# maturk/dn-splatter

Measured on NVIDIA H100. Metric: rendered Mpix/s (fwd+bwd, RGB+depth+normal), higher is better.
Workload: dtype f32

## Files before the change

### dn_splatter_b200/_lib.py

```python
from __future__ import annotations

import ctypes as C
import os
from typing import Optional

HERE = os.path.dirname(os.path.abspath(__file__))
LIB_PATH = os.path.join(HERE, "libdnr_b200.so")

FLAG_ACTIVATED, FLAG_ANTIALIASED, FLAG_NORMALS, FLAG_ACCUMULATE, FLAG_EXACT_LISTS = 1, 2, 4, 8, 16
FLAG_HOST_CAMERA = 32
FLAG_PERSISTENT_WS = 256
LOSS_FUSED_BWD, LOSS_IMG_U8, LOSS_NORMAL_U8, LOSS_EDGE_FROM_IMAGE = 1, 2, 4, 8
REC_FLOATS, REC_FLOATS_N, GRAD_FLOATS = 12, 16, 16
DEPTH_LOSS_TYPES = {None: 0, "EdgeAwareLogL1": 1, "LogL1": 2, "L1": 3, "MSE": 4}

_f, _i, _p = C.c_float, C.c_int32, C.c_void_p


class DnrArgs(C.Structure):

    _fields_ = [
        ("n_gauss", _i), ("width", _i), ("height", _i), ("tile_size", _i), ("sh_degree", _i), ("sh_bases", _i),
        ("flags", C.c_uint32), ("list_shift", _i),
        ("near_plane", _f), ("far_plane", _f), ("eps2d", _f), ("radius_clip", _f),
        ("background", _f * 3), ("reserved1", _f),
        ("n_isects", C.c_int64),
        ("viewmat", _p), ("K", _p), ("c2w", _p),
        ("means", _p), ("quats", _p), ("scales", _p), ("opacities", _p), ("sh_dc", _p), ("sh_rest", _p),
        ("radii", _p), ("means2d", _p), ("depths", _p), ("conics", _p), ("opac_act", _p), ("compensations", _p),
        ("colors", _p), ("normals_world", _p), ("tiles_per_gauss", _p), ("depth_keys", _p), ("records", _p), ("cull_lim", _p),
        ("ws_scan", _p), ("ws_sort", _p), ("flatten_ids", _p), ("tile_offsets", _p), ("n_isects_dev", _p),
        ("out_rgb", _p), ("out_depth", _p), ("out_alpha", _p), ("out_normal", _p), ("out_surface_normal", _p),
        ("last_ids", _p), ("normal_norm", _p), ("clamp_mask", _p), ("depth_max", _p),
        ("v_rgb", _p), ("v_depth", _p), ("v_normal", _p), ("v_alpha", _p), ("grad_records", _p),
        ("v_means", _p), ("v_quats", _p), ("v_scales", _p), ("v_opacities", _p), ("v_sh_dc", _p), ("v_sh_rest", _p),
        ("v_means2d", _p), ("v_means2d_abs", _p),
        ("gt_depth", _p), ("gt_normal", _p), ("gt_rgb", _p), ("loss_partials", _p), ("v_loss", _p),
        ("depth_lambda", _f), ("depth_tolerance", _f), ("depth_loss_type", _i), ("use_normal_loss", _i),
        ("host_cam", _f * 32),
        ("reserved2", _p),
        ("loss_flags", C.c_uint32), ("reserved3", _i), ("gt_image", _p), ("v_l1", _p), ("touched", _p), ("stats", _p),
        ("v_viewmat", _p),
    ]


class DnrAdamSeg(C.Structure):

    _fields_ = [("p", _p), ("g", _p), ("m", _p), ("v", _p), ("n", C.c_int64), ("lr", C.c_double), ("eps", C.c_double),
                ("bc1", C.c_double), ("bc2_sqrt", C.c_double), ("dense", C.c_int64)]


class DnrGradSeg(C.Structure):

    _fields_ = [("g", _p), ("width", _i), ("dense", _i)]


PEER_MAX = 8


class DnrPeerReduce(C.Structure):

    _fields_ = [("world", _i), ("rank", _i), ("n_gauss", _i), ("reserved", _i), ("peer_flat", _p * PEER_MAX),
                ("peer_touched", _p * PEER_MAX), ("mask", _p)]


class DnrKnnGrid(C.Structure):

    _fields_ = [("lo", _f * 3), ("cell", _f), ("inv_cell", _f), ("dims", C.c_int32 * 3)]


class DnrTsdfGrid(C.Structure):

    _fields_ = [("origin", _f * 3), ("voxel", _f), ("sdf_trunc", _f), ("dims", C.c_int32 * 3), ("voxels", _p)]


class DnrMcField(C.Structure):

    _fields_ = [("values", _p), ("valid", _p), ("tsdf", _p), ("dims", C.c_int32 * 3), ("iso", _f), ("origin", _f * 3),
                ("spacing", _f)]


class DnrPoissonGrid(C.Structure):

    _fields_ = [("origin", _f * 3), ("cell", _f), ("depth", _i), ("reserved", _i)]


class DnrGridDesc(C.Structure):

    _fields_ = [("origin", _f * 3), ("cell", _f), ("dims", C.c_int32 * 3), ("channels", _i)]


POISSON_MIN_DEPTH, POISSON_MAX_DEPTH, POISSON_MAX_CYCLES = 4, 10, 100


POINTER_FIELDS = {n for n, t in DnrArgs._fields_ if t is _p}

_lib: Optional[C.CDLL] = None

KERNELS_PER_CALL = {
    "dnr_project_fwd": (1, 0), "dnr_bin_scan": (2, 8), "dnr_bin_sort": (3, 4), "dnr_raster_fwd": (1, 0),
    "dnr_finalize_fwd": (1, 0), "dnr_normal_from_depth": (1, 0), "dnr_raster_bwd": (1, 0), "dnr_project_bwd": (1, 0),
    "dnr_loss_fwd": (2, 0), "dnr_loss_bwd": (1, 0), "dnr_scale_loss_fwd": (1, 0), "dnr_scale_loss_bwd": (1, 0),
    "dnr_l1_fwd": (1, 0), "dnr_l1_bwd": (1, 0), "dnr_u8_to_f32": (1, 0),
    "dnr_ssim_fwd": (1, 0), "dnr_ssim_bwd": (1, 0), "dnr_ssim_fwd_ex": (1, 0), "dnr_ssim_bwd_ex": (1, 0), "dnr_photometric_fwd": (2, 0), "dnr_photometric_bwd": (1, 0), "dnr_adam_step": (1, 0), "dnr_adam_step_reduce": (2, 0),
    "dnr_grad_zero": (1, 0),
    "dnr_knn_build": (2, 1), "dnr_knn_query": (1, 0), "dnr_density": (1, 0), "dnr_ray_densities": (1, 0),
    "dnr_tsdf_integrate": (1, 0), "dnr_mc_count": (1, 6), "dnr_mc_emit": (2, 0),
    "dnr_grid_sample": (1, 0), "dnr_mesh_visibility": (1, 0),
}
LAUNCHES = {"handwritten": 0, "cub": 0}
DEBUG_CAPTURE = os.environ.get("DNR_DEBUG_CAPTURE") == "1"


def capture_ok(where: str) -> None:
    if not DEBUG_CAPTURE:
        return
    import torch

    try:
        torch.cuda.is_current_stream_capturing()
    except Exception as exc:
        raise DnrError(f"stream capture invalidated by {where}: {exc}") from exc


class _Counting:

    def __init__(self, lib):
        self._lib = lib

    def __getattr__(self, name):
        fn = getattr(self._lib, name)
        k = KERNELS_PER_CALL.get(name)
        if k is None:
            return fn

        def call(*args):
            LAUNCHES["handwritten"] += k[0]
            LAUNCHES["cub"] += k[1]
            rc = fn(*args)
            if DEBUG_CAPTURE:
                capture_ok(f"{name} (rc {rc})")
            return rc

        self.__dict__[name] = call
        return call


class DnrError(RuntimeError):
    pass


def load():
    global _lib
    if _lib is not None:
        return _lib
    if not os.path.exists(LIB_PATH):
        raise DnrError(
            f"{LIB_PATH} is missing: build it with `python -m dn_splatter_b200.build` "
            "(nvcc, sm_90a). dn_splatter_b200 has no CPU or PyTorch fallback."
        )
    lib = C.CDLL(LIB_PATH)
    A = C.POINTER(DnrArgs)
    lib.dnr_version.restype = C.c_int
    lib.dnr_error_string.restype = C.c_char_p
    lib.dnr_error_string.argtypes = [C.c_int]
    for name in ("dnr_project_fwd", "dnr_bin_sort", "dnr_raster_fwd", "dnr_finalize_fwd", "dnr_normal_from_depth",
                 "dnr_raster_bwd", "dnr_project_bwd", "dnr_loss_fwd"):
        fn = getattr(lib, name)
        fn.restype = C.c_int
        fn.argtypes = [A, C.c_void_p]
    lib.dnr_bin_scan.restype = C.c_int
    lib.dnr_bin_scan.argtypes = [A, C.c_void_p, C.POINTER(C.c_int64)]
    lib.dnr_loss_bwd.restype = C.c_int
    lib.dnr_loss_bwd.argtypes = [A, C.c_void_p, C.c_void_p, C.c_void_p]
    lib.dnr_scale_loss_fwd.restype = C.c_int
    lib.dnr_scale_loss_fwd.argtypes = [C.c_void_p, C.c_int32, C.c_void_p, C.c_void_p]
    lib.dnr_scale_loss_bwd.restype = C.c_int
    lib.dnr_scale_loss_bwd.argtypes = [C.c_void_p, C.c_int32, C.c_void_p, C.c_void_p, C.c_void_p]
    lib.dnr_l1_fwd.restype = C.c_int
    lib.dnr_l1_fwd.argtypes = [C.c_void_p, C.c_void_p, C.c_int64, C.c_int32, C.c_void_p, C.c_void_p]
    lib.dnr_l1_bwd.restype = C.c_int
    lib.dnr_l1_bwd.argtypes = [C.c_void_p, C.c_void_p, C.c_int64, C.c_int32, C.c_void_p, C.c_void_p, C.c_void_p]
    lib.dnr_u8_to_f32.restype = C.c_int
    lib.dnr_u8_to_f32.argtypes = [C.c_void_p, C.c_int64, C.c_float, C.c_float, C.c_void_p, C.c_void_p]
    lib.dnr_ssim_fwd.restype = C.c_int
    lib.dnr_ssim_fwd.argtypes = [C.c_void_p, C.c_void_p, C.c_int32, C.c_int32, C.c_int32, C.c_void_p, C.c_void_p, C.c_void_p]
    lib.dnr_ssim_fwd_ex.restype = C.c_int
    lib.dnr_ssim_fwd_ex.argtypes = [C.c_void_p, C.c_void_p, C.c_int32, C.c_int32, C.c_int32, C.c_int32, C.c_void_p, C.c_void_p,
                                    C.c_void_p]
    lib.dnr_ssim_bwd_ex.restype = C.c_int
    lib.dnr_ssim_bwd_ex.argtypes = [C.c_void_p, C.c_void_p, C.c_int32, C.c_int32, C.c_int32, C.c_int32, C.c_void_p, C.c_void_p,
                                    C.c_void_p, C.c_void_p]
    lib.dnr_photometric_fwd.restype = C.c_int
    lib.dnr_photometric_fwd.argtypes = [C.c_void_p, C.c_void_p, C.c_int32, C.c_int32, C.c_int32, C.c_int32, C.c_float, C.c_void_p,
                                        C.c_void_p, C.c_void_p]
    lib.dnr_photometric_bwd.restype = C.c_int
    lib.dnr_photometric_bwd.argtypes = [C.c_void_p, C.c_void_p, C.c_int32, C.c_int32, C.c_int32, C.c_int32, C.c_float, C.c_void_p,
                                        C.c_void_p, C.c_void_p, C.c_void_p]
    lib.dnr_adam_step.restype = C.c_int
    lib.dnr_adam_step.argtypes = [C.c_void_p, C.c_int32, C.c_double, C.c_double, C.c_void_p]
    lib.dnr_adam_step_reduce.restype = C.c_int
    lib.dnr_adam_step_reduce.argtypes = [C.c_void_p, C.c_void_p, C.c_int32, C.c_double, C.c_double, C.c_void_p, C.c_void_p]
    lib.dnr_grad_zero.restype = C.c_int
    lib.dnr_grad_zero.argtypes = [C.c_void_p, C.c_int32, C.c_void_p, C.c_int32, C.c_void_p]
    lib.dnr_knn_workspace_bytes.restype = C.c_int64
    lib.dnr_knn_workspace_bytes.argtypes = [C.c_int32, C.c_void_p]
    lib.dnr_knn_build.restype = C.c_int
    lib.dnr_knn_build.argtypes = [C.c_void_p, C.c_int32, C.c_void_p, C.c_void_p, C.c_int64, C.c_void_p]
    lib.dnr_knn_query.restype = C.c_int
    lib.dnr_knn_query.argtypes = [C.c_int32, C.c_void_p, C.c_void_p, C.c_void_p, C.c_int32, C.c_int32, C.c_int32, C.c_void_p,
                                  C.c_void_p, C.c_void_p]
    lib.dnr_density.restype = C.c_int
    lib.dnr_density.argtypes = [C.c_void_p, C.c_int64, C.c_void_p, C.c_int32, C.c_int32, C.c_void_p, C.c_void_p, C.c_void_p,
                                C.c_void_p, C.c_int32, C.c_float, C.c_void_p, C.c_void_p]
    lib.dnr_ray_densities.restype = C.c_int
    lib.dnr_ray_densities.argtypes = [C.c_void_p, C.c_int64, C.c_void_p, C.c_int32, C.c_void_p, C.c_void_p, C.c_void_p, C.c_void_p,
                                      C.c_void_p, C.c_int32, C.c_int32, C.c_float, C.c_void_p, C.c_void_p, C.c_void_p, C.c_void_p]
    lib.dnr_tsdf_integrate.restype = C.c_int
    lib.dnr_tsdf_integrate.argtypes = [C.c_void_p, C.c_void_p, C.c_void_p, C.c_void_p, C.c_int32, C.c_int32, C.c_void_p,
                                       C.c_float, C.c_void_p]
    lib.dnr_mc_count_workspace_bytes.restype = C.c_int64
    lib.dnr_mc_count_workspace_bytes.argtypes = [C.c_void_p]
    lib.dnr_mc_count.restype = C.c_int
    lib.dnr_mc_count.argtypes = [C.c_void_p, C.c_void_p, C.c_int64, C.c_void_p, C.c_void_p]
    lib.dnr_mc_emit_workspace_bytes.restype = C.c_int64
    lib.dnr_mc_emit_workspace_bytes.argtypes = [C.c_void_p]
    lib.dnr_mc_emit.restype = C.c_int
    lib.dnr_mc_emit.argtypes = [C.c_void_p, C.c_void_p, C.c_void_p, C.c_void_p, C.c_int64, C.c_void_p, C.c_void_p, C.c_void_p,
                                C.c_void_p]
    lib.dnr_poisson_splat_workspace_bytes.restype = C.c_int64
    lib.dnr_poisson_splat_workspace_bytes.argtypes = [C.c_void_p, C.c_int64]
    lib.dnr_poisson_splat.restype = C.c_int
    lib.dnr_poisson_splat.argtypes = [C.c_void_p, C.c_void_p, C.c_void_p, C.c_void_p, C.c_int64, C.c_void_p, C.c_int64,
                                      C.c_void_p, C.c_void_p, C.c_void_p, C.c_void_p, C.c_void_p, C.c_void_p, C.c_void_p]
    lib.dnr_poisson_solve_workspace_bytes.restype = C.c_int64
    lib.dnr_poisson_solve_workspace_bytes.argtypes = [C.c_void_p, C.c_int32]
    lib.dnr_poisson_solve.restype = C.c_int
    lib.dnr_poisson_solve.argtypes = [C.c_void_p, C.c_void_p, C.c_void_p, C.c_float, C.c_float, C.c_int32, C.c_void_p, C.c_int64,
                                      C.c_void_p, C.c_void_p, C.c_void_p, C.c_void_p]
    lib.dnr_grid_sample.restype = C.c_int
    lib.dnr_grid_sample.argtypes = [C.c_void_p, C.c_void_p, C.c_void_p, C.c_int64, C.c_void_p, C.c_void_p]
    lib.dnr_mesh_depth_workspace_bytes.restype = C.c_int64
    lib.dnr_mesh_depth_workspace_bytes.argtypes = [C.c_int64]
    lib.dnr_mesh_depth.restype = C.c_int
    lib.dnr_mesh_depth.argtypes = [C.c_void_p, C.c_int32, C.c_void_p, C.c_int64, C.c_void_p, C.c_int32, C.c_int32, C.c_int32,
                                   C.c_float, C.c_float, C.c_void_p, C.c_int64, C.c_void_p, C.c_void_p]
    lib.dnr_mesh_visibility.restype = C.c_int
    lib.dnr_mesh_visibility.argtypes = [C.c_void_p, C.c_int64, C.c_void_p, C.c_void_p, C.c_void_p, C.c_int32, C.c_int32, C.c_int32,
                                        C.c_float, C.c_void_p, C.c_void_p, C.c_void_p]
    lib.dnr_ssim_bwd.restype = C.c_int
    lib.dnr_ssim_bwd.argtypes = [C.c_void_p, C.c_void_p, C.c_int32, C.c_int32, C.c_int32, C.c_void_p, C.c_void_p, C.c_void_p,
                                 C.c_void_p]
    lib.dnr_bin_scan_workspace_bytes.restype = C.c_size_t
    lib.dnr_bin_scan_workspace_bytes.argtypes = [C.c_int32]
    lib.dnr_bin_sort_workspace_bytes.restype = C.c_size_t
    lib.dnr_bin_sort_workspace_bytes.argtypes = [C.c_int32, C.c_int64, C.c_int32]
    _lib = _Counting(lib)
    return _lib


EXPORTS = (
    "dnr_version", "dnr_error_string", "dnr_project_fwd", "dnr_bin_scan_workspace_bytes", "dnr_bin_scan",
    "dnr_bin_sort_workspace_bytes", "dnr_bin_sort", "dnr_raster_fwd", "dnr_finalize_fwd", "dnr_normal_from_depth",
    "dnr_raster_bwd", "dnr_project_bwd", "dnr_loss_fwd", "dnr_loss_bwd", "dnr_scale_loss_fwd", "dnr_scale_loss_bwd",
    "dnr_l1_fwd", "dnr_l1_bwd", "dnr_u8_to_f32", "dnr_ssim_fwd", "dnr_ssim_bwd", "dnr_ssim_fwd_ex", "dnr_ssim_bwd_ex", "dnr_photometric_fwd", "dnr_photometric_bwd", "dnr_adam_step", "dnr_adam_step_reduce", "dnr_grad_zero", "dnr_knn_workspace_bytes", "dnr_knn_build", "dnr_knn_query",
    "dnr_density", "dnr_ray_densities", "dnr_tsdf_integrate", "dnr_mc_count_workspace_bytes", "dnr_mc_count",
    "dnr_mc_emit_workspace_bytes", "dnr_mc_emit", "dnr_poisson_splat_workspace_bytes", "dnr_poisson_splat",
    "dnr_poisson_solve_workspace_bytes", "dnr_poisson_solve", "dnr_grid_sample", "dnr_mesh_depth_workspace_bytes",
    "dnr_mesh_depth", "dnr_mesh_visibility",
)


def check(code: int, what: str) -> None:
    if code != 0:
        msg = load().dnr_error_string(code).decode()
        raise DnrError(f"{what} failed with code {code}: {msg}")
```

### dn_splatter_b200/csrc/binning.cu

```cuda
#include <cub/cub.cuh>
#include <thrust/iterator/transform_iterator.h>

#include "common.cuh"

namespace {

inline size_t align_up(size_t x, size_t a = 256) { return (x + a - 1) / a * a; }

struct ToI64 {
  __host__ __device__ __forceinline__ int64_t operator()(int32_t v) const { return (int64_t)v; }
};

__global__ void iota_kernel(int32_t* out, int32_t n) {
  const int i = blockIdx.x * blockDim.x + threadIdx.x;
  if (i < n) out[i] = i;
}

struct ScanWs {
  uint32_t* keys_sorted;
  int32_t* order;
  int32_t* iota;
  int32_t* counts;
  int64_t* isect_start;
  void* cub_temp;
  size_t cub_bytes;
  size_t total;
};

ScanWs carve_scan(void* base, int32_t n) {
  ScanWs w;
  size_t off = 0;
  char* p = (char*)base;
  w.keys_sorted = (uint32_t*)(p + off); off += align_up((size_t)n * 4);
  w.order = (int32_t*)(p + off); off += align_up((size_t)n * 4);
  w.iota = (int32_t*)(p + off); off += align_up((size_t)n * 4);
  w.counts = (int32_t*)(p + off); off += align_up((size_t)(n + 1) * 4);
  w.isect_start = (int64_t*)(p + off); off += align_up((size_t)(n + 1) * 8);
  size_t sort_bytes = 0, scan_bytes = 0;
  cub::DeviceRadixSort::SortPairs(nullptr, sort_bytes, (const uint32_t*)nullptr, (uint32_t*)nullptr, (const int32_t*)nullptr,
                                  (int32_t*)nullptr, n, 0, 32);
  auto it = thrust::make_transform_iterator((const int32_t*)nullptr, ToI64());
  cub::DeviceScan::ExclusiveSum(nullptr, scan_bytes, it, (int64_t*)nullptr, n + 1);
  w.cub_bytes = sort_bytes > scan_bytes ? sort_bytes : scan_bytes;
  w.cub_temp = (void*)(p + off); off += align_up(w.cub_bytes);
  w.total = off;
  return w;
}

template <typename KeyT>
inline int sort_end_bit(int tile_bits) {
  const int full = (int)(8 * sizeof(KeyT));
  return tile_bits < full ? tile_bits : full;
}

template <typename KeyT>
struct SortWs {
  KeyT* keys_in;
  KeyT* keys_out;
  int32_t* gids_in;
  void* cub_temp;
  size_t cub_bytes;
  size_t total;
};

template <typename KeyT>
SortWs<KeyT> carve_sort(void* base, int64_t n_isects, int tile_bits) {
  SortWs<KeyT> w;
  size_t off = 0;
  char* p = (char*)base;
  const size_t n = (size_t)(n_isects > 0 ? n_isects : 1);
  w.keys_in = (KeyT*)(p + off); off += align_up(n * sizeof(KeyT));
  w.keys_out = (KeyT*)(p + off); off += align_up(n * sizeof(KeyT));
  w.gids_in = (int32_t*)(p + off); off += align_up(n * 4);
  size_t sort_bytes = 0;
  cub::DeviceRadixSort::SortPairs(nullptr, sort_bytes, (const KeyT*)nullptr, (KeyT*)nullptr, (const int32_t*)nullptr,
                                  (int32_t*)nullptr, (int64_t)n, 0, sort_end_bit<KeyT>(tile_bits));
  w.cub_bytes = sort_bytes;
  w.cub_temp = (void*)(p + off); off += align_up(sort_bytes);
  w.total = off;
  return w;
}

inline int tile_bits_for(int n_tiles) {
  int b = 1;
  while ((1 << b) <= n_tiles) ++b;
  return b;
}

struct HitGauss {
  int g, radius, x0, y0, nx, ny;
  float mx, my, A, B, invA, bac, twoAL, ex_max, ey_max, ey_star;
};

__device__ __forceinline__ void list_box(float mx, float my, int radius, int ts, int tiles_x, int tiles_y, int& x0, int& y0,
                                         int& x1, int& y1) {
  if (ts == DNR_TILE) { dnr_tile_box(mx, my, radius, tiles_x, tiles_y, x0, y0, x1, y1); return; }
  const float inv = 1.0f / (float)ts;
  const float r = (float)radius * inv, tcx = mx * inv, tcy = my * inv;
  x0 = min(max((int)floorf(tcx - r), 0), tiles_x);
  y0 = min(max((int)floorf(tcy - r), 0), tiles_y);
  x1 = min(max((int)ceilf(tcx + r), 0), tiles_x);
  y1 = min(max((int)ceilf(tcy + r), 0), tiles_y);
}

__device__ __forceinline__ HitGauss load_hit_gauss(const DnrArgs& a, const int32_t* __restrict__ order, int i, int tiles_x,
                                                   int tiles_y) {
  HitGauss h;
  h.g = 0; h.radius = 0; h.x0 = h.y0 = h.nx = h.ny = 0;
  h.mx = h.my = h.A = h.B = h.invA = h.bac = h.twoAL = h.ex_max = h.ey_max = h.ey_star = 0.f;
  if (i < a.n_gauss) {
    h.g = order[i];
    h.radius = a.radii[h.g];
    if (h.radius > 0) {
      h.mx = a.means2d[h.g * 2 + 0]; h.my = a.means2d[h.g * 2 + 1];
      int x1, y1;
      list_box(h.mx, h.my, h.radius, DNR_TILE << a.list_shift, tiles_x, tiles_y, h.x0, h.y0, x1, y1);
      h.nx = x1 - h.x0;
      h.ny = y1 - h.y0;
      if (!(a.flags & DNR_FLAG_EXACT_LISTS)) {
        const float A = a.conics[h.g * 3 + 0], B = a.conics[h.g * 3 + 1], C = a.conics[h.g * 3 + 2];
        const float L = a.cull_lim[h.g];
        const float det = A * C - B * B;
        if (!(L > 0.f) || !(det > 0.f)) {
          h.ny = 0;
        } else {
          h.A = A; h.B = B; h.invA = 1.0f / A; h.bac = -det; h.twoAL = 2.0f * A * L;
          h.ex_max = sqrtf(2.0f * L * C / det) * 1.0001f + 0.01f;
          h.ey_max = sqrtf(2.0f * L * A / det) * 1.0001f + 0.01f;
          h.ey_star = -B * h.ex_max / C;
        }
      }
    }
  }
  return h;
}

__device__ __forceinline__ void row_span(const HitGauss& h, int ty, bool exact, int ts, int& lo, int& hi) {
  lo = h.x0; hi = h.x0 + h.nx;
  if (exact) return;
  float e0 = ((float)(ty * ts) + 0.5f) - h.my - 0.01f;
  float e1 = ((float)(ty * ts + ts - 1) + 0.5f) - h.my + 0.01f;
  if (e0 > h.ey_max || e1 < -h.ey_max) { hi = lo; return; }
  e0 = fmaxf(e0, -h.ey_max); e1 = fminf(e1, h.ey_max);
  const float s0 = sqrtf(fmaxf(fmaf(h.bac, e0 * e0, h.twoAL), 0.f)), s1 = sqrtf(fmaxf(fmaf(h.bac, e1 * e1, h.twoAL), 0.f));
  float xmax = fmaxf((-h.B * e0 + s0) * h.invA, (-h.B * e1 + s1) * h.invA);
  float xmin = fminf((-h.B * e0 - s0) * h.invA, (-h.B * e1 - s1) * h.invA);
  if (h.ey_star >= e0 && h.ey_star <= e1) xmax = h.ex_max;
  if (-h.ey_star >= e0 && -h.ey_star <= e1) xmin = -h.ex_max;
  xmax = xmax + 0.01f + 1e-5f * fabsf(xmax);
  xmin = xmin - 0.01f - 1e-5f * fabsf(xmin);
  const float inv = 1.0f / (float)ts;
  const int t_lo = (int)ceilf((h.mx + xmin - ((float)ts - 0.5f)) * inv);
  const int t_hi = (int)floorf((h.mx + xmax - 0.5f) * inv) + 1;
  lo = max(lo, t_lo); hi = min(hi, t_hi);
}

__global__ void __launch_bounds__(256) count_kernel(const DnrArgs a, const int32_t* __restrict__ order,
                                                   int32_t* __restrict__ counts, int tiles_x, int tiles_y) {
  const int i = blockIdx.x * blockDim.x + threadIdx.x;
  if (i > a.n_gauss) return;
  const HitGauss h = load_hit_gauss(a, order, i, tiles_x, tiles_y);
  const bool exact = (a.flags & DNR_FLAG_EXACT_LISTS) != 0;
  const int ts = DNR_TILE << a.list_shift;
  int cnt = 0;
  for (int r = 0; r < h.ny; ++r) {
    int lo, hi;
    row_span(h, h.y0 + r, exact, ts, lo, hi);
    cnt += max(hi - lo, 0);
  }
  counts[i] = (i < a.n_gauss) ? cnt : 0;
}

template <typename KeyT>
__global__ void __launch_bounds__(256) emit_kernel(const DnrArgs a, const int32_t* __restrict__ order,
                                                  const int64_t* __restrict__ isect_start, KeyT* __restrict__ keys,
                                                  int32_t* __restrict__ gids, int tiles_x, int tiles_y) {
  const int i = blockIdx.x * blockDim.x + threadIdx.x;
  if (i >= a.n_gauss) return;
  int64_t dst = isect_start[i];
  const int64_t dst_end = isect_start[i + 1];
  if (dst_end <= dst) return;
  const HitGauss h = load_hit_gauss(a, order, i, tiles_x, tiles_y);
  const int64_t cap = a.n_isects;
  const bool exact = (a.flags & DNR_FLAG_EXACT_LISTS) != 0;
  const int ts = DNR_TILE << a.list_shift;
  for (int r = 0; r < h.ny; ++r) {
    int lo, hi;
    row_span(h, h.y0 + r, exact, ts, lo, hi);
    const int row_key = (h.y0 + r) * tiles_x;
    for (int x = lo; x < hi; ++x, ++dst) {
      if (dst < cap) {
        keys[dst] = (KeyT)(row_key + x);
        gids[dst] = h.g;
      }
    }
  }
}

template <typename KeyT>
__global__ void __launch_bounds__(256) pad_kernel(KeyT* __restrict__ keys, int32_t* __restrict__ gids,
                                                 const int64_t* __restrict__ n_isects_dev, int64_t cap, KeyT pad_key) {
  for (int64_t i = *n_isects_dev + (int64_t)blockIdx.x * blockDim.x + threadIdx.x; i < cap; i += (int64_t)gridDim.x * blockDim.x) {
    keys[i] = pad_key;
    gids[i] = 0;
  }
}

template <typename KeyT>
__global__ void __launch_bounds__(256) offsets_kernel(const KeyT* __restrict__ keys, const int64_t* __restrict__ n_isects_dev,
                                                     int64_t cap, int n_tiles, int32_t* __restrict__ offsets) {
  const int64_t i = (int64_t)blockIdx.x * blockDim.x + threadIdx.x;
  const int64_t n_isects = min(*n_isects_dev, cap);
  if (n_isects == 0) {
    if (i <= n_tiles) offsets[i] = 0;
    return;
  }
  if (i >= n_isects) return;
  const int cur = (int)keys[i];
  if (i == 0) {
    for (int t = 0; t <= cur; ++t) offsets[t] = 0;
  } else {
    const int prev = (int)keys[i - 1];
    for (int t = prev + 1; t <= cur; ++t) offsets[t] = (int32_t)i;
  }
  if (i == n_isects - 1) {
    for (int t = cur + 1; t <= n_tiles; ++t) offsets[t] = (int32_t)n_isects;
  }
}

template <typename KeyT>
int bin_sort_impl(const DnrArgs* a, cudaStream_t s, int n_tiles, int tile_bits) {
  const int tiles_x = dnr_stiles_x(a), tiles_y = dnr_stiles_y(a);
  ScanWs sw = carve_scan(a->ws_scan, a->n_gauss);
  const int64_t cap = a->n_isects;
  SortWs<KeyT> w = carve_sort<KeyT>(a->ws_sort, cap, tile_bits);
  if (cap > 0) {
    emit_kernel<KeyT><<<(unsigned)((a->n_gauss + 255) / 256), 256, 0, s>>>(*a, sw.order, sw.isect_start, w.keys_in, w.gids_in,
                                                                          tiles_x, tiles_y);
    DNR_CHECK_LAUNCH();
    pad_kernel<KeyT><<<DNR_NUM_SMS * 2, 256, 0, s>>>(w.keys_in, w.gids_in, a->n_isects_dev, cap, (KeyT)n_tiles);
    DNR_CHECK_LAUNCH();
    size_t bytes = w.cub_bytes;
    const int end_bit = sort_end_bit<KeyT>(tile_bits);
    DNR_CUDA(cub::DeviceRadixSort::SortPairs(w.cub_temp, bytes, (const KeyT*)w.keys_in, w.keys_out,
                                             (const int32_t*)w.gids_in, a->flatten_ids, cap, 0, end_bit, s));
  }
  const int64_t n = cap > (int64_t)n_tiles + 1 ? cap : (int64_t)n_tiles + 1;
  offsets_kernel<KeyT><<<(unsigned)((n + 255) / 256), 256, 0, s>>>(w.keys_out, a->n_isects_dev, cap, n_tiles, a->tile_offsets);
  DNR_CHECK_LAUNCH();
  return 0;
}

}

extern "C" size_t dnr_bin_scan_workspace_bytes(int32_t n_gauss) {
  if (n_gauss <= 0) return 0;
  return carve_scan(nullptr, n_gauss).total;
}

extern "C" int dnr_bin_scan(const DnrArgs* a, void* stream, int64_t* n_isects_host) {
  if (!a) return DNR_E_NULL;
  if (a->n_gauss <= 0 || a->width <= 0 || a->height <= 0) return DNR_E_SIZE;
  if (a->list_shift < 0 || a->list_shift > 3) return DNR_E_OPTION;
  if ((a->flags & DNR_FLAG_EXACT_LISTS) && a->list_shift != 0) return DNR_E_OPTION;
  if (!a->ws_scan || !a->depth_keys || !a->tiles_per_gauss || !a->n_isects_dev || !a->radii || !a->means2d) return DNR_E_NULL;
  if (!(a->flags & DNR_FLAG_EXACT_LISTS) && (!a->conics || !a->cull_lim)) return DNR_E_NULL;
  cudaStream_t s = (cudaStream_t)stream;
  const int32_t n = a->n_gauss;
  ScanWs w = carve_scan(a->ws_scan, n);
  iota_kernel<<<(n + 255) / 256, 256, 0, s>>>(w.iota, n);
  DNR_CHECK_LAUNCH();
  size_t bytes = w.cub_bytes;
  DNR_CUDA(cub::DeviceRadixSort::SortPairs(w.cub_temp, bytes, (const uint32_t*)a->depth_keys, w.keys_sorted,
                                           (const int32_t*)w.iota, w.order, n, 0, 32, s));
  {
    const int64_t threads = (int64_t)n + 1;
    count_kernel<<<(unsigned)((threads + 255) / 256), 256, 0, s>>>(*a, w.order, w.counts, dnr_stiles_x(a), dnr_stiles_y(a));
    DNR_CHECK_LAUNCH();
  }
  auto it = thrust::make_transform_iterator((const int32_t*)w.counts, ToI64());
  bytes = w.cub_bytes;
  DNR_CUDA(cub::DeviceScan::ExclusiveSum(w.cub_temp, bytes, it, w.isect_start, n + 1, s));
  DNR_CUDA(cudaMemcpyAsync(a->n_isects_dev, w.isect_start + n, sizeof(int64_t), cudaMemcpyDeviceToDevice, s));
  if (n_isects_host) {
    int64_t total = 0;
    DNR_CUDA(cudaMemcpyAsync(&total, w.isect_start + n, sizeof(int64_t), cudaMemcpyDeviceToHost, s));
    DNR_CUDA(cudaStreamSynchronize(s));
    *n_isects_host = total;
    if (total > 0x7FFFFFFFLL) return DNR_E_OVERFLOW;
  }
  return 0;
}

extern "C" size_t dnr_bin_sort_workspace_bytes(int32_t n_gauss, int64_t n_isects, int32_t n_tiles) {
  (void)n_gauss;
  if (n_isects < 0 || n_tiles <= 0) return 0;
  const int bits = tile_bits_for(n_tiles);
  if (n_tiles < 65536) return carve_sort<uint16_t>(nullptr, n_isects, bits).total;
  return carve_sort<uint32_t>(nullptr, n_isects, bits).total;
}

extern "C" int dnr_bin_sort(const DnrArgs* a, void* stream) {
  if (!a) return DNR_E_NULL;
  if (a->n_gauss <= 0 || a->n_isects < 0 || a->width <= 0 || a->height <= 0) return DNR_E_SIZE;
  if (a->n_isects > 0x7FFFFFFFLL) return DNR_E_OVERFLOW;
  if (!a->ws_scan || !a->ws_sort || !a->tile_offsets || !a->means2d || !a->radii || !a->n_isects_dev) return DNR_E_NULL;
  if (!(a->flags & DNR_FLAG_EXACT_LISTS) && (!a->conics || !a->cull_lim)) return DNR_E_NULL;
  if (a->n_isects > 0 && !a->flatten_ids) return DNR_E_NULL;
  if (a->list_shift < 0 || a->list_shift > 3) return DNR_E_OPTION;
  if ((a->flags & DNR_FLAG_EXACT_LISTS) && a->list_shift != 0) return DNR_E_OPTION;
  const int n_tiles = dnr_stiles_x(a) * dnr_stiles_y(a);
  const int bits = tile_bits_for(n_tiles);
  cudaStream_t s = (cudaStream_t)stream;
  if (n_tiles < 65536) return bin_sort_impl<uint16_t>(a, s, n_tiles, bits);
  return bin_sort_impl<uint32_t>(a, s, n_tiles, bits);
}
```

Baseline: 786.7.

## Cache depth-sorted gaussian records for emit and fuse padding into emit kernel

The count kernel now writes a packed 32-byte record per visible gaussian, holding mean, conic, cull limit, radius and id, in depth-sorted order. The emit kernel reads these contiguous records instead of gathering scattered per-gaussian arrays through the order permutation. The separate pad kernel is removed, and emit threads now pad the key/id buffers to capacity, which saves one launch. The cost is an extra workspace buffer and record writes in the count pass, and the padding loop now depends on the grid size of the emit launch.

```diff
diff --git a/dn_splatter_b200/_lib.py b/dn_splatter_b200/_lib.py
--- a/dn_splatter_b200/_lib.py
+++ b/dn_splatter_b200/_lib.py
@@ -98,7 +98,7 @@
 _lib: Optional[C.CDLL] = None
 
 KERNELS_PER_CALL = {
-    "dnr_project_fwd": (1, 0), "dnr_bin_scan": (2, 8), "dnr_bin_sort": (3, 4), "dnr_raster_fwd": (1, 0),
+    "dnr_project_fwd": (1, 0), "dnr_bin_scan": (2, 8), "dnr_bin_sort": (2, 4), "dnr_raster_fwd": (1, 0),
     "dnr_finalize_fwd": (1, 0), "dnr_normal_from_depth": (1, 0), "dnr_raster_bwd": (1, 0), "dnr_project_bwd": (1, 0),
     "dnr_loss_fwd": (2, 0), "dnr_loss_bwd": (1, 0), "dnr_scale_loss_fwd": (1, 0), "dnr_scale_loss_bwd": (1, 0),
     "dnr_l1_fwd": (1, 0), "dnr_l1_bwd": (1, 0), "dnr_u8_to_f32": (1, 0),
diff --git a/dn_splatter_b200/csrc/binning.cu b/dn_splatter_b200/csrc/binning.cu
--- a/dn_splatter_b200/csrc/binning.cu
+++ b/dn_splatter_b200/csrc/binning.cu
@@ -11,16 +11,19 @@
   __host__ __device__ __forceinline__ int64_t operator()(int32_t v) const { return (int64_t)v; }
 };
 
-__global__ void iota_kernel(int32_t* out, int32_t n) {
-  const int i = blockIdx.x * blockDim.x + threadIdx.x;
-  if (i < n) out[i] = i;
-}
+struct __align__(16) BinRec {
+  float mx, my, A, B, C, lim;
+  int32_t radius, g;
+};
+static_assert(sizeof(BinRec) == 32, "bin records are two 16-byte loads");
+
 
 struct ScanWs {
   uint32_t* keys_sorted;
   int32_t* order;
   int32_t* iota;
   int32_t* counts;
+  BinRec* recs;
   int64_t* isect_start;
   void* cub_temp;
   size_t cub_bytes;
@@ -35,6 +38,7 @@
   w.order = (int32_t*)(p + off); off += align_up((size_t)n * 4);
   w.iota = (int32_t*)(p + off); off += align_up((size_t)n * 4);
   w.counts = (int32_t*)(p + off); off += align_up((size_t)(n + 1) * 4);
+  w.recs = (BinRec*)(p + off); off += align_up((size_t)n * sizeof(BinRec));
   w.isect_start = (int64_t*)(p + off); off += align_up((size_t)(n + 1) * 8);
   size_t sort_bytes = 0, scan_bytes = 0;
   cub::DeviceRadixSort::SortPairs(nullptr, sort_bytes, (const uint32_t*)nullptr, (uint32_t*)nullptr, (const int32_t*)nullptr,
@@ -103,23 +107,37 @@
   y1 = min(max((int)ceilf(tcy + r), 0), tiles_y);
 }
 
-__device__ __forceinline__ HitGauss load_hit_gauss(const DnrArgs& a, const int32_t* __restrict__ order, int i, int tiles_x,
-                                                   int tiles_y) {
+__device__ __forceinline__ BinRec load_bin_rec(const DnrArgs& a, const int32_t* __restrict__ order, int i) {
+  BinRec r;
+  r.g = order[i];
+  r.radius = a.radii[r.g];
+  r.mx = r.my = r.A = r.B = r.C = r.lim = 0.f;
+  if (r.radius > 0) {
+    r.mx = a.means2d[r.g * 2 + 0]; r.my = a.means2d[r.g * 2 + 1];
+    if (!(a.flags & DNR_FLAG_EXACT_LISTS)) {
+      r.A = a.conics[r.g * 3 + 0]; r.B = a.conics[r.g * 3 + 1]; r.C = a.conics[r.g * 3 + 2];
+      r.lim = a.cull_lim[r.g];
+    }
+  }
+  return r;
+}
+
+__device__ __forceinline__ HitGauss load_hit_gauss(const DnrArgs& a, const BinRec& r, int tiles_x, int tiles_y) {
   HitGauss h;
   h.g = 0; h.radius = 0; h.x0 = h.y0 = h.nx = h.ny = 0;
   h.mx = h.my = h.A = h.B = h.invA = h.bac = h.twoAL = h.ex_max = h.ey_max = h.ey_star = 0.f;
-  if (i < a.n_gauss) {
-    h.g = order[i];
-    h.radius = a.radii[h.g];
+  {
+    h.g = r.g;
+    h.radius = r.radius;
     if (h.radius > 0) {
-      h.mx = a.means2d[h.g * 2 + 0]; h.my = a.means2d[h.g * 2 + 1];
+      h.mx = r.mx; h.my = r.my;
       int x1, y1;
       list_box(h.mx, h.my, h.radius, DNR_TILE << a.list_shift, tiles_x, tiles_y, h.x0, h.y0, x1, y1);
       h.nx = x1 - h.x0;
       h.ny = y1 - h.y0;
       if (!(a.flags & DNR_FLAG_EXACT_LISTS)) {
-        const float A = a.conics[h.g * 3 + 0], B = a.conics[h.g * 3 + 1], C = a.conics[h.g * 3 + 2];
-        const float L = a.cull_lim[h.g];
+        const float A = r.A, B = r.B, C = r.C;
+        const float L = r.lim;
         const float det = A * C - B * B;
         if (!(L > 0.f) || !(det > 0.f)) {
           h.ny = 0;
@@ -155,54 +173,65 @@
   lo = max(lo, t_lo); hi = min(hi, t_hi);
 }
 
+__global__ void iota_kernel(int32_t* out, int32_t n) {
+  const int i = blockIdx.x * blockDim.x + threadIdx.x;
+  if (i < n) out[i] = i;
+}
+
 __global__ void __launch_bounds__(256) count_kernel(const DnrArgs a, const int32_t* __restrict__ order,
-                                                   int32_t* __restrict__ counts, int tiles_x, int tiles_y) {
+                                                   BinRec* __restrict__ recs, int32_t* __restrict__ counts, int tiles_x,
+                                                   int tiles_y) {
   const int i = blockIdx.x * blockDim.x + threadIdx.x;
   if (i > a.n_gauss) return;
-  const HitGauss h = load_hit_gauss(a, order, i, tiles_x, tiles_y);
-  const bool exact = (a.flags & DNR_FLAG_EXACT_LISTS) != 0;
-  const int ts = DNR_TILE << a.list_shift;
+  if (i == a.n_gauss) {
+    counts[i] = 0;
+    return;
+  }
+  const BinRec r = load_bin_rec(a, order, i);
   int cnt = 0;
-  for (int r = 0; r < h.ny; ++r) {
-    int lo, hi;
-    row_span(h, h.y0 + r, exact, ts, lo, hi);
-    cnt += max(hi - lo, 0);
-  }
-  counts[i] = (i < a.n_gauss) ? cnt : 0;
-}
-
-template <typename KeyT>
-__global__ void __launch_bounds__(256) emit_kernel(const DnrArgs a, const int32_t* __restrict__ order,
+  if (r.radius > 0) {
+    recs[i] = r;
+    const HitGauss h = load_hit_gauss(a, r, tiles_x, tiles_y);
+    const bool exact = (a.flags & DNR_FLAG_EXACT_LISTS) != 0;
+    const int ts = DNR_TILE << a.list_shift;
+    for (int row = 0; row < h.ny; ++row) {
+      int lo, hi;
+      row_span(h, h.y0 + row, exact, ts, lo, hi);
+      cnt += max(hi - lo, 0);
+    }
+  }
+  counts[i] = cnt;
+}
+
+template <typename KeyT>
+__global__ void __launch_bounds__(256) emit_kernel(const DnrArgs a, const BinRec* __restrict__ recs,
                                                   const int64_t* __restrict__ isect_start, KeyT* __restrict__ keys,
-                                                  int32_t* __restrict__ gids, int tiles_x, int tiles_y) {
+                                                  int32_t* __restrict__ gids, int tiles_x, int tiles_y, KeyT pad_key) {
   const int i = blockIdx.x * blockDim.x + threadIdx.x;
-  if (i >= a.n_gauss) return;
-  int64_t dst = isect_start[i];
-  const int64_t dst_end = isect_start[i + 1];
-  if (dst_end <= dst) return;
-  const HitGauss h = load_hit_gauss(a, order, i, tiles_x, tiles_y);
   const int64_t cap = a.n_isects;
-  const bool exact = (a.flags & DNR_FLAG_EXACT_LISTS) != 0;
-  const int ts = DNR_TILE << a.list_shift;
-  for (int r = 0; r < h.ny; ++r) {
-    int lo, hi;
-    row_span(h, h.y0 + r, exact, ts, lo, hi);
-    const int row_key = (h.y0 + r) * tiles_x;
-    for (int x = lo; x < hi; ++x, ++dst) {
-      if (dst < cap) {
-        keys[dst] = (KeyT)(row_key + x);
-        gids[dst] = h.g;
+  if (i < a.n_gauss) {
+    int64_t dst = isect_start[i];
+    const int64_t dst_end = isect_start[i + 1];
+    if (dst_end > dst) {
+      const HitGauss h = load_hit_gauss(a, recs[i], tiles_x, tiles_y);
+      const bool exact = (a.flags & DNR_FLAG_EXACT_LISTS) != 0;
+      const int ts = DNR_TILE << a.list_shift;
+      for (int r = 0; r < h.ny; ++r) {
+        int lo, hi;
+        row_span(h, h.y0 + r, exact, ts, lo, hi);
+        const int row_key = (h.y0 + r) * tiles_x;
+        for (int x = lo; x < hi; ++x, ++dst) {
+          if (dst < cap) {
+            keys[dst] = (KeyT)(row_key + x);
+            gids[dst] = h.g;
+          }
+        }
       }
     }
   }
-}
-
-template <typename KeyT>
-__global__ void __launch_bounds__(256) pad_kernel(KeyT* __restrict__ keys, int32_t* __restrict__ gids,
-                                                 const int64_t* __restrict__ n_isects_dev, int64_t cap, KeyT pad_key) {
-  for (int64_t i = *n_isects_dev + (int64_t)blockIdx.x * blockDim.x + threadIdx.x; i < cap; i += (int64_t)gridDim.x * blockDim.x) {
-    keys[i] = pad_key;
-    gids[i] = 0;
+  for (int64_t j = isect_start[a.n_gauss] + i; j < cap; j += (int64_t)gridDim.x * blockDim.x) {
+    keys[j] = pad_key;
+    gids[j] = 0;
   }
 }
 
@@ -235,10 +264,8 @@
   const int64_t cap = a->n_isects;
   SortWs<KeyT> w = carve_sort<KeyT>(a->ws_sort, cap, tile_bits);
   if (cap > 0) {
-    emit_kernel<KeyT><<<(unsigned)((a->n_gauss + 255) / 256), 256, 0, s>>>(*a, sw.order, sw.isect_start, w.keys_in, w.gids_in,
-                                                                          tiles_x, tiles_y);
-    DNR_CHECK_LAUNCH();
-    pad_kernel<KeyT><<<DNR_NUM_SMS * 2, 256, 0, s>>>(w.keys_in, w.gids_in, a->n_isects_dev, cap, (KeyT)n_tiles);
+    emit_kernel<KeyT><<<(unsigned)((a->n_gauss + 255) / 256), 256, 0, s>>>(*a, sw.recs, sw.isect_start, w.keys_in, w.gids_in,
+                                                                          tiles_x, tiles_y, (KeyT)n_tiles);
     DNR_CHECK_LAUNCH();
     size_t bytes = w.cub_bytes;
     const int end_bit = sort_end_bit<KeyT>(tile_bits);
@@ -275,7 +302,8 @@
                                            (const int32_t*)w.iota, w.order, n, 0, 32, s));
   {
     const int64_t threads = (int64_t)n + 1;
-    count_kernel<<<(unsigned)((threads + 255) / 256), 256, 0, s>>>(*a, w.order, w.counts, dnr_stiles_x(a), dnr_stiles_y(a));
+    count_kernel<<<(unsigned)((threads + 255) / 256), 256, 0, s>>>(*a, w.order, w.recs, w.counts, dnr_stiles_x(a),
+                                                                   dnr_stiles_y(a));
     DNR_CHECK_LAUNCH();
   }
   auto it = thrust::make_transform_iterator((const int32_t*)w.counts, ToI64());
```

Result: no change. 791.3 (median of 6 runs) (+0.6%).
